# kaftanski/fissure-segmentation

Hardware: AMD Instinct MI355X
Metric: points/sec fwd+bwd DGCNN-seg N=2048 k=20 (higher is better)
Workload: dtype f32

## Files before the change

fissure-segmentation_amd/csrc/edgeconv.hip:

```cpp
#include <type_traits>

#include "edgeconv_internal.h"
#include "knn_internal.h"

namespace {

constexpr int TP = 16;
constexpr int FSG_CSR_SPLIT = 16;
constexpr int TPW = 2;

__global__ __launch_bounds__(1024) void csr_build_kernel(const int32_t *__restrict__ idx, int N, int k,
                                                          int32_t *__restrict__ rowptr, int32_t *__restrict__ col) {
    extern __shared__ int sh[];
    int *hist = sh;
    int *part = sh + N;
    const int b = blockIdx.x, tid = threadIdx.x;
    const long NK = (long)N * k;
    const int32_t *ib = idx + b * NK;
    for (int j = tid; j < N; j += 1024) hist[j] = 0;
    __syncthreads();
    for (long e0 = tid; e0 < NK; e0 += 8 * 1024) {
        int dst[8];
#pragma unroll
        for (int u = 0; u < 8; ++u) dst[u] = (e0 + u * 1024 < NK) ? ib[e0 + u * 1024] : -1;
// ... 380 lines not shown
        cm += red2[2][s2][ch];
    }
    const double mu = n > 0.0 ? bm / n : 0.0;
    double M2 = n > 0.0 ? cm - bm * mu : 0.0;
    M2 = M2 > 0.0 ? M2 : 0.0;
    const double var = n > 0.0 ? M2 / n : 0.0;
    mean_out[c] = (float)mu;
    invstd_out[c] = (float)(1.0 / sqrt(var + (double)eps));
    if (running_mean) {
        const double unbiased = n > 1.0 ? M2 / (n - 1.0) : var;
        running_mean[c] = (float)((1.0 - momentum) * running_mean[c] + momentum * mu);
        running_var[c] = (float)((1.0 - momentum) * running_var[c] + momentum * unbiased);
    }
}

__global__ __launch_bounds__(256) void ec1_apply_kernel(const float *__restrict__ ysel, const float *__restrict__ gamma,
                                                         const float *__restrict__ beta, const float *__restrict__ mean,
                                                         const float *__restrict__ invstd, int N, int Co, float slope,
                                                         float *__restrict__ out, float *__restrict__ out_pm) {
    __shared__ float tile[64][65];
    const int b = blockIdx.x, i0 = blockIdx.y * 64, cg = blockIdx.z;
    const int lane = threadIdx.x & 63, wave = __builtin_amdgcn_readfirstlane(threadIdx.x >> 6);
    const int c = cg * 64 + lane;
    const float g = gamma[c] * invstd[c], sh = beta[c] - mean[c] * g;
    float yv[16];
#pragma unroll
    for (int u = 0; u < 16; ++u) yv[u] = ysel[((long)b * N + min(i0 + wave + 4 * u, N - 1)) * Co + c];
#pragma unroll
    for (int u = 0; u < 16; ++u) {
        const int p = wave + 4 * u, i = i0 + p;
// ... 175 lines not shown
    };
    if (i0 + 64 <= N) rows(std::false_type{});
    else rows(std::true_type{});
    red[0][wave][lane] = sb;
    red[1][wave][lane] = sg;
    __syncthreads();
    if (wave == 0) {
        const long rec = (long)b * gridDim.y + blockIdx.y;
        float *pr = partials + rec * 2 * Co;
        pr[c] = red[0][0][lane] + red[0][1][lane] + red[0][2][lane] + red[0][3][lane];
        pr[Co + c] = red[1][0][lane] + red[1][1][lane] + red[1][2][lane] + red[1][3][lane];
    }
}

constexpr int SUMP_CH = 16, SUMP_SLICES = 64;
__global__ __launch_bounds__(SUMP_CH * SUMP_SLICES) void sum_partials_kernel(const float *__restrict__ partials, int R, int Co,
                                                                             int nvec, float *__restrict__ out0,
                                                                             float *__restrict__ out1) {
    __shared__ double red[SUMP_SLICES][SUMP_CH];
    const int ch = threadIdx.x & (SUMP_CH - 1), slice = threadIdx.x / SUMP_CH;
    const int c = blockIdx.x * SUMP_CH + ch, v = blockIdx.y;
    double acc = 0.0;
    for (int r0 = slice; r0 < R; r0 += 4 * SUMP_SLICES) {
        float t[4];
#pragma unroll
        for (int u = 0; u < 4; ++u) t[u] = partials[((long)min(r0 + u * SUMP_SLICES, R - 1) * nvec + v) * Co + c];
#pragma unroll
        for (int u = 0; u < 4; ++u)
            if (r0 + u * SUMP_SLICES < R) acc += t[u];
    }
    red[slice][ch] = acc;
    __syncthreads();
    if (slice < 8) {
        double t = 0.0;
#pragma unroll
        for (int w = 0; w < 8; ++w) t += red[8 * slice + w][ch];
        red[8 * slice][ch] = t;
    }
    __syncthreads();
    if (slice == 0) {
        double t = 0.0;
#pragma unroll
        for (int w = 0; w < 8; ++w) t += red[8 * w][ch];
        (v == 0 ? out0 : out1)[c] = (float)t;
    }
}

__global__ __launch_bounds__(256) void ec1_bwd_gather_kernel(
    const float *__restrict__ pq, const int32_t *__restrict__ rowptr, const int32_t *__restrict__ col,
    const float *__restrict__ h, const uint8_t *__restrict__ arg, const float *__restrict__ ssum,
    const float *__restrict__ gamma, const float *__restrict__ mean, const float *__restrict__ invstd,
    const float *__restrict__ dbeta, const float *__restrict__ dgamma, int N, int k, int Co, int training, float invM,
    float *__restrict__ grad_pq) {
    typedef f32x2 f2;
    typedef f32x4 f4;
    __shared__ float comb[4][2][4][64];
    const int b = blockIdx.x, cg = blockIdx.z;
    const int lane = threadIdx.x & 63, wave = __builtin_amdgcn_readfirstlane(threadIdx.x >> 6);
    const int j = blockIdx.y * 4 + wave;
    if (j >= N) return;
// ... 64 lines not shown
}

}

int fsg_ec_stats1_records(int B, int N) { return B * fsg_cdiv(N, TP * TPW); }

int fsg_ec_stats1_launch(const float *pq, const int32_t *idx, const float *gamma, int B, int N, int k, int Co,
                         float *ysel, uint8_t *arg, float *ssum, float *partials, hipStream_t st) {
    FSG_REQUIRE((long)N * 2 * Co * 4 < (1L << 31), "edgeconv/stats: a cloud's [P | Q] rows must stay below 2 GiB (N=%d, Co=%d)", N, Co);
    hipLaunchKernelGGL(ec1_stats_select_kernel<false>, dim3(B, fsg_cdiv(N, TP * TPW), Co / 64), dim3(256 * TPW), 0, st, pq, idx,
                       gamma, N, k, Co, 1, ysel, arg, ssum, partials);
    FSG_CHECK_LAUNCH("edgeconv/stats");
    return FSG_OK;
}

size_t fsg_ec_finalize_stage_floats(int Co) { return (size_t)FIN_S * 3 * Co * 2 + 2; }

int fsg_ec_finalize_launch(const float *partials, int R, int Co, float eps, float momentum, float *mean, float *invstd,
                           float *running_mean, float *running_var, hipStream_t st) {
    hipLaunchKernelGGL(bn_finalize_kernel, dim3(Co / FIN_CH), dim3(FIN_CH * FIN_SL), 0, st, partials, R, Co, eps, momentum, mean, invstd,
                       running_mean, running_var);
    FSG_CHECK_LAUNCH("edgeconv/finalize");
    return FSG_OK;
}

int fsg_ec_apply_prep_launch(const float *ysel, const float *gamma, const float *beta, const float *mean, const float *invstd,
                             int B, int N, int Co, float slope, float *out, float *out_pm, void *knn_ws, size_t knn_ws_bytes,
                             const float *w_next, float *pq_next, hipStream_t st) {
    float *xx, *xs, *cscale;
    void *cand;
// ... 237 lines not shown
```

fissure-segmentation_amd/csrc/edgeconv2.hip:

```cpp

#include "edgeconv_internal.h"

namespace {

__device__ __forceinline__ bf16x8 pack8(const float (&v)[8]) {
    bf16x8 r;
#pragma unroll
    for (int i = 0; i < 8; ++i) r[i] = (__bf16)v[i];
    return r;
}

constexpr int C1 = 64;
constexpr int LD1 = C1 + 1;
constexpr int MAXPAIR = 3;

struct Tile {
    int TP, R, Rpad;
};

template <int C2, bool BF>
__global__ __launch_bounds__(256) void ec2_fwd_kernel(const float *__restrict__ pq, const int32_t *__restrict__ idx,
                                                       const float *__restrict__ w2, const float *__restrict__ gamma1,
                                                       const float *__restrict__ beta1, const float *__restrict__ mean1,
                                                       const float *__restrict__ invstd1,
// ... 1060 lines not shown
        { int RTb, TPb, Gb; ec2s_tiling(k, B, N, false, true, RTb, TPb, Gb); if (Gb > Gs) Gs = Gb; }
        if (Gs > G) G = Gs;
    }
    const size_t rec1 = (size_t)fsg_ec_stats1_records(B, N) * 3 * C1 + fsg_ec_finalize_stage_floats(C1);
    const size_t rec2 = (size_t)B * G * 3 * C2 + fsg_ec_finalize_stage_floats(C2);
    const size_t scratch1 = (size_t)B * N * C1 * sizeof(float) + (size_t)B * N * C1;
    return sizeof(float) * (rec1 + rec2) + scratch1 + 256;
}

static int ec2_fwd_impl(bool bf16, const float *pq, const int32_t *idx, const float *w2, const float *gamma1,
                                     const float *beta1, float *running_mean1, float *running_var1, const float *gamma2,
                                     const float *beta2, float *running_mean2, float *running_var2, int B, int N, int k,
                                     int C2, int training, float momentum1, float momentum2, float eps1, float eps2,
                                     float slope, float *out, float *out_pm, float *ssum1, float *mean1, float *invstd1,
                                     float *ysel2, uint8_t *arg2, float *ssum2, float *mean2, float *invstd2,
                                     void *workspace, fsg_stream_t stream) {
    FSG_REQUIRE(pq && idx && w2 && gamma1 && beta1 && gamma2 && beta2 && mean1 && invstd1 && ysel2 && arg2 &&
                    mean2 && invstd2 && workspace,
                "fsg_edgeconv2_fwd_f32: NULL pointer");
    FSG_REQUIRE(B > 0 && N > 0 && N <= (1 << 21) && k > 0 && k <= 64 && (C2 == 64 || C2 == 128) && B <= 65535,
                "fsg_edgeconv2_fwd_f32: bad shape B=%d N=%d k=%d C2=%d (layer widths 64 -> 64|128 only, N <= 2^21)", B, N, k, C2);
    FSG_REQUIRE(!training || (ssum1 && ssum2), "fsg_edgeconv2_fwd_f32: training needs ssum1/ssum2");
    hipStream_t st = (hipStream_t)stream;
    int TP, Rpad, G;
    ec2_tiling(k, C2, TP, Rpad, G, B, N);
    int RTs = 0, TPs = 0, Gs = 0, Gws = G;
    if (ec2_split(C2)) {
        ec2s_tiling(k, B, N, false, bf16, RTs, TPs, Gs);
        if (Gs > Gws) Gws = Gs;
    }
    const int rec1 = fsg_ec_stats1_records(B, N);
    float *part1 = (float *)workspace;
    float *part2 = part1 + (size_t)rec1 * 3 * C1 + fsg_ec_finalize_stage_floats(C1);
    float *ysel1 = part2 + (size_t)B * Gws * 3 * C2 + fsg_ec_finalize_stage_floats(C2);
    uint8_t *arg1 = (uint8_t *)(ysel1 + (size_t)B * N * C1);
    int rc;
    if (training) {
        if ((rc = fsg_ec_stats1_launch(pq, idx, gamma1, B, N, k, C1, ysel1, arg1, ssum1, part1, st)) != FSG_OK) return rc;
        if ((rc = fsg_ec_finalize_launch(part1, rec1, C1, eps1, momentum1, mean1, invstd1, running_mean1, running_var1,
                                         st)) != FSG_OK)
            return rc;
    }
    const size_t lds = sizeof(float) * ((size_t)C2 * LD1 + (size_t)Rpad * (C2 + 1) + 3 * 4 * C2);
#define FSG_EC2_FWD(CC, BFX)                                                                                             \
    do {                                                                                                                 \
        FSG_GRANT_LDS("fsg_edgeconv2_fwd", (ec2_fwd_kernel<CC, BFX>), FSG_LDS_WHOLE_CU);                             \
        hipLaunchKernelGGL((ec2_fwd_kernel<CC, BFX>), dim3(B, G), dim3(256), lds, st, pq, idx, w2, gamma1, beta1, mean1,    \
                           invstd1, gamma2, N, k, TP, Rpad, training, slope, ysel2, arg2, ssum2, part2);                 \
    } while (0)
#define FSG_EC2S_FWD(NPX, RTX)                                                                                            \
    do {                                                                                                                 \
        FSG_GRANT_LDS("fsg_edgeconv2_fwd", (ec2s_fwd_kernel<NPX, RTX>), FSG_LDS_WHOLE_CU);                           \
// ... 24 lines not shown
                                     int C2, int training, float momentum1, float momentum2, float eps1, float eps2,
                                     float slope, float *out, float *out_pm, float *ssum1, float *mean1, float *invstd1,
                                     float *ysel2, uint8_t *arg2, float *ssum2, float *mean2, float *invstd2,
                                     void *workspace, fsg_stream_t stream) {
    return ec2_fwd_impl(false, pq, idx, w2, gamma1, beta1, running_mean1, running_var1, gamma2, beta2, running_mean2, running_var2, B, N, k, C2, training, momentum1, momentum2, eps1, eps2, slope, out, out_pm, ssum1, mean1, invstd1, ysel2, arg2, ssum2, mean2, invstd2, workspace, stream);
}

extern "C" int fsg_edgeconv2_fwd_bf16(const float *pq, const int32_t *idx, const float *w2, const float *gamma1,
                                     const float *beta1, float *running_mean1, float *running_var1, const float *gamma2,
                                     const float *beta2, float *running_mean2, float *running_var2, int B, int N, int k,
                                     int C2, int training, float momentum1, float momentum2, float eps1, float eps2,
                                     float slope, float *out, float *out_pm, float *ssum1, float *mean1, float *invstd1,
                                     float *ysel2, uint8_t *arg2, float *ssum2, float *mean2, float *invstd2,
                                     void *workspace, fsg_stream_t stream) {
    return ec2_fwd_impl(true, pq, idx, w2, gamma1, beta1, running_mean1, running_var1, gamma2, beta2, running_mean2, running_var2, B, N, k, C2, training, momentum1, momentum2, eps1, eps2, slope, out, out_pm, ssum1, mean1, invstd1, ysel2, arg2, ssum2, mean2, invstd2, workspace, stream);
}

static void ec2_bwd_tiling(int k, int C2, int &TP, int &Rpad, int &G, int B, int N) {
    TP = 64 / k;
    if (TP < 1) TP = 1;
    Rpad = (TP * k + 31) & ~31;
    const int ntiles = (N + TP - 1) / TP;
    G = 768 / (B > 0 ? B : 1);
    if (G < 1) G = 1;
    if (G > ntiles) G = ntiles;
}

extern "C" size_t fsg_edgeconv2_bwd_workspace_bytes(int B, int N, int k, int C2) {
    int TP, Rpad, G;
    ec2_bwd_tiling(k, C2, TP, Rpad, G, B, N);
// ... 58 lines not shown
        FSG_GRANT_LDS("fsg_edgeconv2_bwd_f32", (ec2s_bwd_kernel<NPX, RTX>), FSG_LDS_WHOLE_CU);                       \
        hipLaunchKernelGGL((ec2s_bwd_kernel<NPX, RTX>), dim3(B, G), dim3(256), ec2s_bwd_lds(NPX, RTX, TPs), st, pq, idx,   \
                           w2, gamma1, beta1, mean1, invstd1, gamma2, mean2, invstd2, grad_beta2, grad_gamma2, h2, arg2, \
                           N, k, TPs, training, invM, slope, du1, dw_part, p1_part);                                     \
    } while (0)
    if (ec2_split(C2)) {
        G = Gs;
        FSG_REQUIRE(ec2s_bwd_lds(bf16 ? 1 : 3, RTs, TPs) <= FSG_LDS_WHOLE_CU, "fsg_edgeconv2_bwd: k=%d needs too much LDS", k);
        if (bf16) { if (RTs == 4) FSG_EC2S_BWD(1, 4); else FSG_EC2S_BWD(1, 2); }
        else { if (RTs == 4) FSG_EC2S_BWD(3, 4); else FSG_EC2S_BWD(3, 2); }
    } else if (C2 == 64) { if (bf16) FSG_EC2_BWD(64, true); else FSG_EC2_BWD(64, false); }
    else { if (bf16) FSG_EC2_BWD(128, true); else FSG_EC2_BWD(128, false); }
#undef FSG_EC2_BWD
#undef FSG_EC2S_BWD
    FSG_CHECK_LAUNCH("fsg_edgeconv2_bwd_f32/mlp");
    if ((rc = fsg_ec_sum_launch(dw_part, B * G, C2 * C1, 1, grad_w2, nullptr, st)) != FSG_OK) return rc;
    if ((rc = fsg_ec_sum_launch(p1_part, B * G, C1, 2, grad_beta1, grad_gamma1, st)) != FSG_OK) return rc;
    hipLaunchKernelGGL(ec2_bwd_gather_kernel, dim3(B, fsg_cdiv(N, 4)), dim3(256), 0, st, pq, rowptr, col, du1, ssum1,
                       gamma1, mean1, invstd1, grad_beta1, grad_gamma1, N, k, training, invM, grad_pq);
    FSG_CHECK_LAUNCH("fsg_edgeconv2_bwd_f32/gather");
    return FSG_OK;
}

extern "C" int fsg_edgeconv2_bwd_f32(const float *grad_out, const float *grad_out_pm, int64_t ld_pm, const float *grad_out_pm2,
                                     int64_t ld_pm2, const float *pq, const int32_t *idx,
                                     const int32_t *rowptr, const int32_t *col, const float *w2, const float *gamma1,
                                     const float *beta1, const float *mean1, const float *invstd1, const float *ssum1,
                                     const float *gamma2, const float *beta2, const float *mean2, const float *invstd2,
                                     const float *ysel2, const uint8_t *arg2, int B, int N, int k, int C2, int training,
                                     float slope, float *grad_pq, float *grad_w2, float *grad_gamma1, float *grad_beta1,
                                     float *grad_gamma2, float *grad_beta2, void *workspace, fsg_stream_t stream) {
    return ec2_bwd_impl(false, grad_out, grad_out_pm, ld_pm, grad_out_pm2, ld_pm2, pq, idx, rowptr, col, w2, gamma1, beta1, mean1, invstd1, ssum1, gamma2, beta2, mean2, invstd2, ysel2, arg2, B, N, k, C2, training, slope, grad_pq, grad_w2, grad_gamma1, grad_beta1, grad_gamma2, grad_beta2, workspace, stream);
// ... 13 lines not shown
```

fissure-segmentation_amd/csrc/edgeconv_internal.h:

```cpp
#pragma once
#include "fsg_common.h"

int fsg_ec_stats1_records(int B, int N);
int fsg_ec_stats1_launch(const float *pq, const int32_t *idx, const float *gamma, int B, int N, int k, int Co,
                         float *ysel, uint8_t *arg, float *ssum, float *partials, hipStream_t st);
int fsg_ec_apply_launch(const float *ysel, const float *gamma, const float *beta, const float *mean, const float *invstd,
                        int B, int N, int Co, float slope, float *out, float *out_pm, hipStream_t st);
int fsg_ec_apply_prep_launch(const float *ysel, const float *gamma, const float *beta, const float *mean, const float *invstd,
                             int B, int N, int Co, float slope, float *out, float *out_pm, void *knn_ws, size_t knn_ws_bytes,
                             const float *w_next, float *pq_next, hipStream_t st);
int fsg_ec_bwd_point_launch(const float *gout, const float *gout_pm, long ld_pm, const float *gout_pm2, long ld_pm2,
                            const float *ysel, const float *gamma, const float *beta, const float *mean, const float *invstd,
                            int B, int N, int Co, float slope, float *h, float *partials, float *dbeta, float *dgamma,
                            hipStream_t st);

size_t fsg_ec_finalize_stage_floats(int Co);
int fsg_ec_finalize_launch(const float *partials, int R, int Co, float eps, float momentum, float *mean, float *invstd,
                           float *running_mean, float *running_var, hipStream_t st);
int fsg_ec_sum_launch(const float *partials, int R, int L, int nvec, float *out0, float *out1, hipStream_t st);

int fsg_csr_bipartite_launch(const int32_t *idx, int B, int NS, int N, int k, int32_t *rowptr, int32_t *col, int32_t *cnt,
                             int32_t *tmp, hipStream_t st);
```

fissure-segmentation_amd/functional.py:

```python
import contextlib as _contextlib
import ctypes
import os as _os

import torch

from . import _lib


def _need_gpu(*tensors):
    for t in tensors:
        if t is not None and not t.is_cuda:
            raise RuntimeError("fissure_segmentation_amd runs on the GPU only (got a CPU tensor); "
                               "the CPU restatement lives in oracle/ and is test infrastructure")


def _p(t):
    return ctypes.c_void_p(t.data_ptr() if t is not None else 0)


def _stream():
    return ctypes.c_void_p(torch.cuda.current_stream().cuda_stream)


def _f32c(t):
# ... 856 lines not shown
        w_cat = _EdgeWeights.apply(conv_weight.reshape(Co, C2).to(torch.float32))
    if x_pm is None:
        x_pm = x.transpose(1, 2)
    if pq_given is not None:
        pq = _LinearPMGiven.apply(x_pm.to(torch.float32), w_cat, pq_given)
    else:
        pq = linear_pm(x_pm.to(torch.float32).contiguous(), w_cat)
    bn_args = _bn_args(bn)
    if idx.dtype != torch.int32:
        idx = idx.to(torch.int32)
    idx = idx.contiguous()
    res = _EdgeConv1.apply(pq, idx, *bn_args, float(slope), knn_ws, w_next if knn_ws is not None else None)
    return _edgeconv_outputs(res, both, w_next is not None)


class _EdgeConv2(torch.autograd.Function):
    @staticmethod
    @_amp_fwd
    def forward(ctx, pq, idx, w2, g1, b1, rm1, rv1, g2, b2, rm2, rv2, training, mom1, mom2, eps1, eps2, slope, knn_ws=None,
                w_next=None):
        pq, w2 = _f32c(pq), _f32c(w2)
        g1, b1, g2, b2 = _f32c(g1), _f32c(b1), _f32c(g2), _f32c(b2)
        B, N, _ = pq.shape
        C2, k, dev = w2.shape[0], idx.shape[2], pq.device

        def new(*shape, dtype=torch.float32):
            return torch.empty(*shape, dtype=dtype, device=dev)
        out, out_pm = new(B, C2, N), new(B, N, C2)
        ysel2, arg2 = new(B, N, C2), new(B, N, C2, dtype=torch.uint8)
        if training:
            ssum1, ssum2 = new(B, N, 64), new(B, N, C2)
            mean1, invstd1, mean2, invstd2 = new(64), new(64), new(C2), new(C2)
        else:
            ssum1 = ssum2 = None
            mean1, invstd1 = _bn_eval_stats(rm1, rv1, eps1)
            mean2, invstd2 = _bn_eval_stats(rm2, rv2, eps2)
        ws = _lib.workspace("fsg_edgeconv2", B, N, k, C2, device=dev)
        t = bool(training)
        ctx.bf16 = bf16_operands()
        with torch.cuda.device(dev):
            _lib.call("fsg_edgeconv2_fwd_bf16" if ctx.bf16 else "fsg_edgeconv2_fwd_f32", _p(pq), _p(idx), _p(w2), _p(g1), _p(b1),
                      _p(rm1 if t else None),
                      _p(rv1 if t else None), _p(g2), _p(b2), _p(rm2 if t else None), _p(rv2 if t else None), B, N, k, C2,
                      int(t), mom1, mom2, eps1, eps2, slope, _p(None if knn_ws is not None else out), _p(out_pm), _p(ssum1), _p(mean1),
                      _p(invstd1), _p(ysel2), _p(arg2), _p(ssum2), _p(mean2), _p(invstd2), _p(ws), _stream())
            pq_next = _apply_pass(ysel2, g2, b2, mean2, invstd2, B, N, C2, slope, out, out_pm, knn_ws, w_next)
        ctx.save_for_backward(pq, idx, w2, g1, b1, mean1, invstd1, ssum1, g2, b2, mean2, invstd2, ysel2, arg2)
        ctx.meta = (B, N, k, C2, t, slope)
        ctx.set_materialize_grads(False)
        if pq_next is None:
            return out, out_pm, out_pm.view(B, N, C2)
        ctx.mark_non_differentiable(pq_next)
        return out, out_pm, out_pm.view(B, N, C2), pq_next

    @staticmethod
    @_amp_bwd
    def backward(ctx, g, g_pm, g_pm2, _g_pq_next=None):
        pq, idx, w2, g1, b1, mean1, invstd1, ssum1, g2, b2, mean2, invstd2, ysel2, arg2 = ctx.saved_tensors
        B, N, k, C2, training, slope = ctx.meta
        dev = pq.device
        g = _f32c(g) if g is not None else None
        g_pm, ld1 = _pm_grad(g_pm, B, N, C2)
        g_pm2, ld2 = _pm_grad(g_pm2, B, N, C2)
        rowptr, col = reverse_graph(idx)
        gpq, gw2 = torch.empty_like(pq), torch.empty_like(w2)
        dg1, db1 = torch.empty_like(g1), torch.empty_like(b1)
        dg2, db2 = torch.empty_like(g2), torch.empty_like(b2)
        ws = _lib.workspace("fsg_edgeconv2_bwd", B, N, k, C2, device=dev)
        with torch.cuda.device(dev):
            _lib.call("fsg_edgeconv2_bwd_bf16" if ctx.bf16 else "fsg_edgeconv2_bwd_f32", _p(g), _p(g_pm), ld1, _p(g_pm2), ld2,
                      _p(pq), _p(idx), _p(rowptr), _p(col),
                      _p(w2), _p(g1),
                      _p(b1), _p(mean1), _p(invstd1), _p(ssum1), _p(g2), _p(b2), _p(mean2), _p(invstd2), _p(ysel2),
                      _p(arg2), B, N, k, C2, int(training), slope, _p(gpq), _p(gw2), _p(dg1), _p(db1), _p(dg2), _p(db2),
                      _p(ws), _stream())
        return (gpq, None, gw2, dg1, db1, None, None, dg2, db2) + (None,) * 10


def edgeconv2_supported(c_mid, c_out, k):
    return c_mid == 64 and c_out in (64, 128) and k <= 64


def _edgeconv_outputs(res, both, want_pq_next):
    out, out_pm, out_pm2 = res[:3]
    pq_next = res[3] if len(res) > 3 else None
    if both == "twice":
        r = (out, out_pm, out_pm2)
    elif both:
        r = (out, out_pm)
    else:
        r = (out,)
# ... 11 lines not shown
        w_cat = _EdgeWeights.apply(conv1_weight.reshape(C1, CC).to(torch.float32))
    if x_pm is None:
        x_pm = x.transpose(1, 2)
    if pq_given is not None:
        pq = _LinearPMGiven.apply(x_pm.to(torch.float32), w_cat, pq_given)
    else:
        pq = linear_pm(x_pm.to(torch.float32).contiguous(), w_cat)
    w2 = conv2_weight.reshape(conv2_weight.shape[0], C1)
    t1, m1 = _bn_step(bn1)
    t2, m2 = _bn_step(bn2)
    if t1 != t2:
        raise RuntimeError("edgeconv2: both BatchNorm layers must be in the same mode")
    if idx.dtype != torch.int32:
        idx = idx.to(torch.int32)
    idx = idx.contiguous()
    res = _EdgeConv2.apply(pq, idx, w2, bn1.weight, bn1.bias, bn1.running_mean, bn1.running_var,
                           bn2.weight, bn2.bias, bn2.running_mean, bn2.running_var, t1, m1, m2,
                           float(bn1.eps), float(bn2.eps), float(slope), knn_ws, w_next if knn_ws is not None else None)
    return _edgeconv_outputs(res, both, w_next is not None)


def pw_weight_image(w, scale=1.0, out=None, ks0=0, KS=None):
    _need_gpu(w)
    N, K = w.shape
    ks = (K + 15) // 16
    KS = ks if KS is None else KS
    if out is None:
        out = torch.empty(((N + 31) // 32) * KS * 3 * 1024, dtype=torch.uint8, device=w.device)
    with torch.cuda.device(w.device):
        _lib.call("fsg_pw_weight_image_f32", _p(w), w.stride(0), w.stride(1), N, K, float(scale), ks0, KS, _p(out), _stream())
    return out


# ... 3163 lines not shown
```

include/fsg_hip.h:

```cpp
#ifndef FSG_HIP_H
#define FSG_HIP_H

#include <stddef.h>
#include <stdint.h>

#ifdef __cplusplus
extern "C" {
#endif

#define FSG_OK 0
#define FSG_ERR_ARG 1
#define FSG_ERR_HIP 2
#define FSG_ERR_UNSUPPORTED 3

#define FSG_KNN_FIX_DIAG 1
#define FSG_KNN_DROP_FIRST 2

#define FSG_KNN_FORCE_ROWS 4

#define FSG_KNN_FORCE_MFMA 8
#define FSG_KNN_DBG_HALF_CHUNKS (1 << 11)
#define FSG_KNN_DBG_TWO_PHASE (1 << 21)
#define FSG_KNN_DBG_ALL_SLOW (1 << 22)
#define FSG_KNN_DBG_STATS (1 << 25)
// ... 96 lines not shown
int fsg_edgeconv2_bwd_f32(const float *grad_out, const float *grad_out_pm, int64_t ld_pm, const float *grad_out_pm2,
                          int64_t ld_pm2, const float *pq, const int32_t *idx,
                          const int32_t *rowptr, const int32_t *col, const float *w2, const float *gamma1,
                          const float *beta1, const float *mean1, const float *invstd1, const float *ssum1,
                          const float *gamma2, const float *beta2, const float *mean2, const float *invstd2,
                          const float *ysel2, const uint8_t *arg2, int B, int N, int k, int C2, int training,
                          float slope, float *grad_pq, float *grad_w2, float *grad_gamma1, float *grad_beta1,
                          float *grad_gamma2, float *grad_beta2, void *workspace, fsg_stream_t stream);
int fsg_edgeconv2_fwd_bf16(const float *pq, const int32_t *idx, const float *w2, const float *gamma1,
                           const float *beta1, float *running_mean1, float *running_var1, const float *gamma2,
                           const float *beta2, float *running_mean2, float *running_var2, int B, int N, int k, int C2,
                           int training, float momentum1, float momentum2, float eps1, float eps2, float slope,
                           float *out, float *out_pm, float *ssum1, float *mean1, float *invstd1, float *ysel2,
                           uint8_t *arg2, float *ssum2, float *mean2, float *invstd2, void *workspace,
                           fsg_stream_t stream);
int fsg_edgeconv2_bwd_bf16(const float *grad_out, const float *grad_out_pm, int64_t ld_pm, const float *grad_out_pm2,
                           int64_t ld_pm2, const float *pq, const int32_t *idx,
                           const int32_t *rowptr, const int32_t *col, const float *w2, const float *gamma1,
                           const float *beta1, const float *mean1, const float *invstd1, const float *ssum1,
                           const float *gamma2, const float *beta2, const float *mean2, const float *invstd2,
                           const float *ysel2, const uint8_t *arg2, int B, int N, int k, int C2, int training,
                           float slope, float *grad_pq, float *grad_w2, float *grad_gamma1, float *grad_beta1,
                           float *grad_gamma2, float *grad_beta2, void *workspace, fsg_stream_t stream);

size_t fsg_bn_act_workspace_bytes(long M, int C);
int fsg_bn_act_fwd_f32(const float *y, const float *gamma, const float *beta, float *running_mean, float *running_var,
                       long M, int C, int training, float momentum, float eps, float slope, float *out, float *mean,
                       float *invstd, float *workspace, fsg_stream_t stream);
int fsg_bn_act_bwd_f32(const float *grad_out, const float *y, const float *gamma, const float *beta, const float *mean,
                       const float *invstd, long M, int C, int training, float slope, float *grad_y, float *grad_gamma,
// ... 511 lines not shown
```

Measured before the change: 18.33 million.

## Compute first EdgeConv BN stats from raw-input moments instead of edge features

For the first EdgeConv layer with at most 4 input channels, batch-norm mean and variance are now derived analytically from first and second moments of the raw coordinates over neighbour edges, folded through the linear weights, instead of being reduced over the full 64-channel edge features. A new moments kernel accumulates these moments in double precision (optionally staging the cloud in LDS) and also writes the per-point neighbour sums, and a single-block fold kernel produces mean, invstd and running stats. Separately, the backward partial-sum launches are merged into one paired kernel. This trades a wide channel reduction for a small moment computation, but relies on BN input being exactly linear in x and adds a single-block serial fold.

```diff
diff --git a/fissure-segmentation_amd/csrc/edgeconv.hip b/fissure-segmentation_amd/csrc/edgeconv.hip
--- a/fissure-segmentation_amd/csrc/edgeconv.hip
+++ b/fissure-segmentation_amd/csrc/edgeconv.hip
@@ -418,6 +418,264 @@
     }
 }
 
+constexpr int MOM_THREADS = 256, MOM_LPP = 4, MOM_PTS = MOM_THREADS / MOM_LPP;
+constexpr int MOM_NM = 44;
+constexpr int MOM_ROW = 23;
+constexpr int MOM_FOLD = 11 * MOM_NM + MOM_NM;
+__constant__ unsigned char MOM_IA[MOM_NM] = {0, 1, 2, 3, 18, 19, 20, 21, 4, 5, 6, 7, 8, 9, 10, 11, 12, 13,
+                                             0, 0, 0, 0, 1, 1, 1, 1, 2, 2, 2, 2, 3, 3, 3, 3,
+                                             18, 18, 18, 18, 19, 19, 19, 20, 20, 21};
+__constant__ unsigned char MOM_IB[MOM_NM] = {22, 22, 22, 22, 22, 22, 22, 22, 22, 22, 22, 22, 22, 22, 22, 22, 22, 22,
+                                             14, 15, 16, 17, 14, 15, 16, 17, 14, 15, 16, 17, 14, 15, 16, 17,
+                                             14, 15, 16, 17, 15, 16, 17, 16, 17, 17};
+__device__ __forceinline__ int mom_tri(int a, int b) {
+    return a * 4 - a * (a - 1) / 2 + (b - a);
+}
+
+struct MomentFold {
+    const float *w_cat;
+    int C, R;
+    double edges, inv_edges, k;
+    float eps, momentum;
+    float *mean, *invstd, *running_mean, *running_var;
+};
+
+__device__ __forceinline__ void ec2_moments_fold(const MomentFold &F, const double *rec, double *sh) {
+    typedef double f64x2 __attribute__((ext_vector_type(2)));
+    const int t = threadIdx.x, pm = t % 22, q = t / 22;
+    float wf[8] = {0.f, 0.f, 0.f, 0.f, 0.f, 0.f, 0.f, 0.f}, rm0 = 0.f, rv0 = 0.f;
+    if (t < 64) {
+#pragma unroll
+        for (int a = 0; a < 4; ++a) {
+            const float wa = F.w_cat[(long)t * F.C + min(a, F.C - 1)], wb = F.w_cat[(long)(64 + t) * F.C + min(a, F.C - 1)];
+            wf[a] = a < F.C ? wa : 0.f;
+            wf[4 + a] = a < F.C ? wb : 0.f;
+        }
+        if (F.running_mean) {
+            rm0 = F.running_mean[t];
+            rv0 = F.running_var[t];
+        }
+    }
+    if (q < 11) {
+        double a0 = 0.0, a1 = 0.0;
+        const int r0 = (int)((long)F.R * q / 11), r1 = (int)((long)F.R * (q + 1) / 11);
+        constexpr int RB = 24;
+        for (int r = r0; r < r1; r += RB) {
+            f64x2 v[RB];
+#pragma unroll
+            for (int u = 0; u < RB; ++u)
+                v[u] = *reinterpret_cast<const f64x2 *>(rec + (long)min(r + u, r1 - 1) * MOM_NM + 2 * pm);
+#pragma unroll
+            for (int u = 0; u < RB; ++u)
+                if (r + u < r1) {
+                    a0 += v[u][0];
+                    a1 += v[u][1];
+                }
+        }
+        sh[q * MOM_NM + 2 * pm] = a0;
+        sh[q * MOM_NM + 2 * pm + 1] = a1;
+    }
+    __syncthreads();
+    if (t < MOM_NM) {
+        double a = 0.0;
+#pragma unroll
+        for (int u = 0; u < 11; ++u) a += sh[u * MOM_NM + t];
+        sh[11 * MOM_NM + t] = a;
+    }
+    __syncthreads();
+    if (t >= 64) return;
+    const double *tot = sh + 11 * MOM_NM;
+    const int c = t;
+    double w[8], mf[8];
+#pragma unroll
+    for (int a = 0; a < 4; ++a) {
+        w[a] = (double)wf[a];
+        w[4 + a] = (double)wf[4 + a];
+        mf[a] = tot[a] * F.inv_edges;
+        mf[4 + a] = F.k * tot[4 + a] * F.inv_edges;
+    }
+    double mu = 0.0, var = 0.0;
+#pragma unroll
+    for (int a = 0; a < 8; ++a) mu += w[a] * mf[a];
+#pragma unroll
+    for (int a = 0; a < 8; ++a)
+#pragma unroll
+        for (int b = 0; b < 8; ++b) {
+            double sff;
+            if (a < 4 && b < 4) sff = tot[8 + mom_tri(min(a, b), max(a, b))];
+            else if (a >= 4 && b >= 4) sff = F.k * tot[34 + mom_tri(min(a, b) - 4, max(a, b) - 4)];
+            else sff = tot[18 + 4 * min(a, b) + (max(a, b) - 4)];
+            var += w[a] * w[b] * (sff * F.inv_edges - mf[a] * mf[b]);
+        }
+    var = var > 0.0 ? var : 0.0;
+    F.mean[c] = (float)mu;
+    F.invstd[c] = (float)(1.0 / sqrt(var + (double)F.eps));
+    if (F.running_mean) {
+        const double n = F.edges, unbiased = n > 1.0 ? var * n / (n - 1.0) : var;
+        F.running_mean[c] = (float)((1.0 - F.momentum) * rm0 + F.momentum * mu);
+        F.running_var[c] = (float)((1.0 - F.momentum) * rv0 + F.momentum * unbiased);
+    }
+}
+
+constexpr size_t MOM_LDS_FIXED = sizeof(double) * (MOM_THREADS * MOM_ROW + 4 * 64);
+template <bool STAGE>
+__global__ __launch_bounds__(MOM_THREADS) void ec2_moments_kernel(const float *__restrict__ x, long sb, long sc,
+                                                                  const int32_t *__restrict__ idx,
+                                                                  const float *__restrict__ pq, int N, int k,
+                                                                  float *__restrict__ ssum, double *__restrict__ rec,
+                                                                  const MomentFold F) {
+    typedef f32x4 f4;
+    extern __shared__ __align__(16) unsigned char mom_lds[];
+    double(*row)[MOM_ROW] = reinterpret_cast<double(*)[MOM_ROW]>(mom_lds);
+    double *red = reinterpret_cast<double *>(mom_lds) + MOM_THREADS * MOM_ROW;
+    f4 *cx = reinterpret_cast<f4 *>(mom_lds + MOM_LDS_FIXED);
+    int32_t *ids = reinterpret_cast<int32_t *>(cx + N);
+    const int tid = threadIdx.x, b = blockIdx.y, i0 = blockIdx.x * MOM_PTS, C = F.C;
+    const int p = tid / MOM_LPP, h = tid % MOM_LPP, i = i0 + p;
+    const bool live = i < N;
+    const float *xb = x + (long)b * sb;
+    const int c16 = tid & 15, pg = tid >> 4;
+    const float *qb = pq + (long)b * N * 128 + 64 + 4 * c16;
+    f4 qv[MOM_PTS / 16];
+#pragma unroll
+    for (int u = 0; u < MOM_PTS / 16; ++u) qv[u] = *reinterpret_cast<const f4 *>(qb + (long)min(i0 + 16 * u + pg, N - 1) * 128);
+    float wpf[4][4];
+#pragma unroll
+    for (int e = 0; e < 4; ++e)
+#pragma unroll
+        for (int a = 0; a < 4; ++a) {
+            const float wv = F.w_cat[(long)(4 * c16 + e) * C + min(a, C - 1)];
+            wpf[e][a] = a < C ? wv : 0.f;
+        }
+    double s[4] = {0.0, 0.0, 0.0, 0.0}, T[10] = {0.0, 0.0, 0.0, 0.0, 0.0, 0.0, 0.0, 0.0, 0.0, 0.0};
+    float xi[4] = {0.f, 0.f, 0.f, 0.f};
+    auto add = [&](const float (&v)[4]) {
+        int t = 0;
+#pragma unroll
+        for (int a = 0; a < 4; ++a) {
+            s[a] += (double)v[a];
+#pragma unroll
+            for (int c = a; c < 4; ++c, ++t) T[t] += (double)v[a] * (double)v[c];
+        }
+    };
+    if (STAGE) {
+        constexpr int ICH = MOM_PTS * 64 / MOM_THREADS;
+        constexpr int SCH = 8;
+        const int cnt = min(MOM_PTS, N - i0) * k;
+        const int32_t *it = idx + ((long)b * N + i0) * k;
+        int32_t idv[ICH];
+#pragma unroll
+        for (int u = 0; u < ICH; ++u) idv[u] = tid + u * MOM_THREADS < cnt ? it[tid + u * MOM_THREADS] : 0;
+        for (int n0 = 0; n0 < N; n0 += SCH * MOM_THREADS) {
+            f4 cv[SCH];
+#pragma unroll
+            for (int u = 0; u < SCH; ++u) {
+                const int n = min(n0 + u * MOM_THREADS + tid, N - 1);
+#pragma unroll
+                for (int c = 0; c < 4; ++c) {
+                    const float xv = xb[min(c, C - 1) * sc + n];
+                    cv[u][c] = c < C ? xv : 0.f;
+                }
+            }
+#pragma unroll
+            for (int u = 0; u < SCH; ++u)
+                if (n0 + u * MOM_THREADS + tid < N) cx[n0 + u * MOM_THREADS + tid] = cv[u];
+        }
+#pragma unroll
+        for (int u = 0; u < ICH; ++u)
+            if (tid + u * MOM_THREADS < cnt) ids[tid + u * MOM_THREADS] = idv[u];
+        __syncthreads();
+        if (live) {
+            const f4 v = cx[i];
+#pragma unroll
+            for (int c = 0; c < 4; ++c) xi[c] = v[c];
+#pragma unroll 4
+            for (int sl = h; sl < k; sl += MOM_LPP) {
+                const f4 vj = cx[min(max(ids[p * k + sl], 0), N - 1)];
+                const float xj[4] = {vj[0], vj[1], vj[2], vj[3]};
+                add(xj);
+            }
+        }
+    } else if (live) {
+#pragma unroll
+        for (int c = 0; c < 4; ++c) {
+            const float xv = xb[min(c, C - 1) * sc + i];
+            xi[c] = c < C ? xv : 0.f;
+        }
+        const int32_t *ib = idx + ((long)b * N + i) * k;
+        constexpr int RB = 5;
+        for (int s0 = h; s0 < k; s0 += MOM_LPP * RB) {
+            int j[RB];
+            float xj[RB][4];
+#pragma unroll
+            for (int u = 0; u < RB; ++u) j[u] = min(max(ib[min(s0 + MOM_LPP * u, k - 1)], 0), N - 1);
+#pragma unroll
+            for (int u = 0; u < RB; ++u)
+#pragma unroll
+                for (int c = 0; c < 4; ++c) {
+                    const float xv = xb[min(c, C - 1) * sc + j[u]];
+                    xj[u][c] = c < C ? xv : 0.f;
+                }
+#pragma unroll
+            for (int u = 0; u < RB; ++u)
+                if (s0 + MOM_LPP * u < k) add(xj[u]);
+        }
+    }
+#pragma unroll
+    for (int a = 0; a < 4; ++a) {
+        row[tid][a] = s[a];
+        row[tid][14 + a] = (double)xi[a];
+        row[tid][18 + a] = h == 0 ? (double)xi[a] : 0.0;
+    }
+#pragma unroll
+    for (int t = 0; t < 10; ++t) row[tid][4 + t] = T[t];
+    row[tid][22] = live ? 1.0 : 0.0;
+    __syncthreads();
+    {
+        const int m = tid & 63, q = tid >> 6;
+        double acc = 0.0;
+        if (m < MOM_NM) {
+            const int ia = MOM_IA[m], ibb = MOM_IB[m];
+#pragma unroll 8
+            for (int l = 64 * q; l < 64 * q + 64; ++l) acc += row[l][ia] * row[l][ibb];
+        }
+        red[q * 64 + m] = acc;
+    }
+    __syncthreads();
+    const long r = (long)b * gridDim.x + blockIdx.x;
+    if (tid < MOM_NM) rec[r * MOM_NM + tid] = ((red[tid] + red[64 + tid]) + red[128 + tid]) + red[192 + tid];
+    {
+        float *sb_out = ssum + (long)b * N * 64 + 4 * c16;
+#pragma unroll
+        for (int u = 0; u < MOM_PTS / 16; ++u) {
+            const int pp = 16 * u + pg;
+            if (i0 + pp < N) {
+                double si[4];
+#pragma unroll
+                for (int a = 0; a < 4; ++a) {
+                    si[a] = row[MOM_LPP * pp][a];
+#pragma unroll
+                    for (int l = 1; l < MOM_LPP; ++l) si[a] += row[MOM_LPP * pp + l][a];
+                }
+                f4 o;
+#pragma unroll
+                for (int e = 0; e < 4; ++e) {
+                    double v = (double)k * (double)qv[u][e];
+#pragma unroll
+                    for (int a = 0; a < 4; ++a) v += (double)wpf[e][a] * si[a];
+                    o[e] = (float)v;
+                }
+                *reinterpret_cast<f4 *>(sb_out + (long)(i0 + pp) * 64) = o;
+            }
+        }
+    }
+}
+
+__global__ __launch_bounds__(MOM_THREADS) void ec2_moments_fold_kernel(const double *__restrict__ rec, const MomentFold F) {
+    __shared__ double red[MOM_FOLD];
+    ec2_moments_fold(F, rec, red);
+}
+
 __global__ __launch_bounds__(256) void ec1_apply_kernel(const float *__restrict__ ysel, const float *__restrict__ gamma,
                                                          const float *__restrict__ beta, const float *__restrict__ mean,
                                                          const float *__restrict__ invstd, int N, int Co, float slope,
@@ -623,36 +881,50 @@
 }
 
 constexpr int SUMP_CH = 16, SUMP_SLICES = 64;
+__device__ __forceinline__ void sum_partials_block(const float *__restrict__ partials, int R, int Co, int nvec,
+                                                   float *__restrict__ out0, float *__restrict__ out1, int bx, int v) {
+    __shared__ double red[SUMP_SLICES][SUMP_CH];
+    const int ch = threadIdx.x & (SUMP_CH - 1), slice = threadIdx.x / SUMP_CH;
+    const int c = bx * SUMP_CH + ch;
+    double acc = 0.0;
+    for (int r0 = slice; r0 < R; r0 += 4 * SUMP_SLICES) {
+        float t[4];
+#pragma unroll
+        for (int u = 0; u < 4; ++u) t[u] = partials[((long)min(r0 + u * SUMP_SLICES, R - 1) * nvec + v) * Co + c];
+#pragma unroll
+        for (int u = 0; u < 4; ++u)
+            if (r0 + u * SUMP_SLICES < R) acc += t[u];
+    }
+    red[slice][ch] = acc;
+    __syncthreads();
+    if (slice < 8) {
+        double t = 0.0;
+#pragma unroll
+        for (int w = 0; w < 8; ++w) t += red[8 * slice + w][ch];
+        red[8 * slice][ch] = t;
+    }
+    __syncthreads();
+    if (slice == 0) {
+        double t = 0.0;
+#pragma unroll
+        for (int w = 0; w < 8; ++w) t += red[8 * w][ch];
+        (v == 0 ? out0 : out1)[c] = (float)t;
+    }
+}
+
 __global__ __launch_bounds__(SUMP_CH * SUMP_SLICES) void sum_partials_kernel(const float *__restrict__ partials, int R, int Co,
                                                                              int nvec, float *__restrict__ out0,
                                                                              float *__restrict__ out1) {
-    __shared__ double red[SUMP_SLICES][SUMP_CH];
-    const int ch = threadIdx.x & (SUMP_CH - 1), slice = threadIdx.x / SUMP_CH;
-    const int c = blockIdx.x * SUMP_CH + ch, v = blockIdx.y;
-    double acc = 0.0;
-    for (int r0 = slice; r0 < R; r0 += 4 * SUMP_SLICES) {
-        float t[4];
-#pragma unroll
-        for (int u = 0; u < 4; ++u) t[u] = partials[((long)min(r0 + u * SUMP_SLICES, R - 1) * nvec + v) * Co + c];
-#pragma unroll
-        for (int u = 0; u < 4; ++u)
-            if (r0 + u * SUMP_SLICES < R) acc += t[u];
-    }
-    red[slice][ch] = acc;
-    __syncthreads();
-    if (slice < 8) {
-        double t = 0.0;
-#pragma unroll
-        for (int w = 0; w < 8; ++w) t += red[8 * slice + w][ch];
-        red[8 * slice][ch] = t;
-    }
-    __syncthreads();
-    if (slice == 0) {
-        double t = 0.0;
-#pragma unroll
-        for (int w = 0; w < 8; ++w) t += red[8 * w][ch];
-        (v == 0 ? out0 : out1)[c] = (float)t;
-    }
+    sum_partials_block(partials, R, Co, nvec, out0, out1, blockIdx.x, blockIdx.y);
+}
+
+__global__ __launch_bounds__(SUMP_CH * SUMP_SLICES) void sum_partials_pair_kernel(
+    const float *__restrict__ pa, int Ra, int La, float *__restrict__ out_a, const float *__restrict__ pb, int Rb, int Lb,
+    float *__restrict__ out_b0, float *__restrict__ out_b1) {
+    const int na = La / SUMP_CH, nb = Lb / SUMP_CH;
+    const int bx = blockIdx.x;
+    if (bx < na) sum_partials_block(pa, Ra, La, 1, out_a, nullptr, bx, 0);
+    else sum_partials_block(pb, Rb, Lb, 2, out_b0, out_b1, (bx - na) % nb, (bx - na) / nb);
 }
 
 __global__ __launch_bounds__(256) void ec1_bwd_gather_kernel(
@@ -747,6 +1019,38 @@
     return FSG_OK;
 }
 
+size_t fsg_ec_moments1_record_bytes(int B, int N) { return (size_t)B * fsg_cdiv(N, MOM_PTS) * MOM_NM * sizeof(double); }
+
+int fsg_ec_moments1_launch(const float *x, long sb, long sc, int C, const int32_t *idx, const float *w_cat, const float *pq, int B,
+                           int N, int k, float eps, float momentum, float *ssum, float *mean, float *invstd, float *running_mean,
+                           float *running_var, void *records, hipStream_t st) {
+    const dim3 grid(fsg_cdiv(N, MOM_PTS), B);
+    const double edges = (double)B * (double)N * (double)k;
+    const MomentFold F{w_cat, C, (int)(grid.x * grid.y), edges, 1.0 / edges, (double)k, eps, momentum,
+                       mean, invstd, running_mean, running_var};
+    const size_t staged = MOM_LDS_FIXED + 16 * (size_t)N + 4 * (size_t)MOM_PTS * k;
+    if (staged <= FSG_LDS_WHOLE_CU) {
+        FSG_GRANT_LDS("fsg_edgeconv2_fwd_moments", ec2_moments_kernel<true>, staged);
+        hipLaunchKernelGGL(ec2_moments_kernel<true>, grid, dim3(MOM_THREADS), staged, st, x, sb, sc, idx, pq, N, k, ssum,
+                           (double *)records, F);
+    } else {
+        hipLaunchKernelGGL(ec2_moments_kernel<false>, grid, dim3(MOM_THREADS), MOM_LDS_FIXED, st, x, sb, sc, idx, pq, N, k, ssum,
+                           (double *)records, F);
+    }
+    FSG_CHECK_LAUNCH("edgeconv2/moments");
+    hipLaunchKernelGGL(ec2_moments_fold_kernel, dim3(1), dim3(MOM_THREADS), 0, st, (const double *)records, F);
+    FSG_CHECK_LAUNCH("edgeconv2/moments_fold");
+    return FSG_OK;
+}
+
+int fsg_ec_sum_pair_launch(const float *pa, int Ra, int La, float *out_a, const float *pb, int Rb, int Lb, float *out_b0,
+                           float *out_b1, hipStream_t st) {
+    hipLaunchKernelGGL(sum_partials_pair_kernel, dim3(La / SUMP_CH + 2 * (Lb / SUMP_CH)), dim3(SUMP_CH * SUMP_SLICES), 0, st, pa, Ra,
+                       La, out_a, pb, Rb, Lb, out_b0, out_b1);
+    FSG_CHECK_LAUNCH("edgeconv/sum_pair");
+    return FSG_OK;
+}
+
 size_t fsg_ec_finalize_stage_floats(int Co) { return (size_t)FIN_S * 3 * Co * 2 + 2; }
 
 int fsg_ec_finalize_launch(const float *partials, int R, int Co, float eps, float momentum, float *mean, float *invstd,
diff --git a/fissure-segmentation_amd/csrc/edgeconv2.hip b/fissure-segmentation_amd/csrc/edgeconv2.hip
--- a/fissure-segmentation_amd/csrc/edgeconv2.hip
+++ b/fissure-segmentation_amd/csrc/edgeconv2.hip
@@ -1098,7 +1098,8 @@
                                      int C2, int training, float momentum1, float momentum2, float eps1, float eps2,
                                      float slope, float *out, float *out_pm, float *ssum1, float *mean1, float *invstd1,
                                      float *ysel2, uint8_t *arg2, float *ssum2, float *mean2, float *invstd2,
-                                     void *workspace, fsg_stream_t stream) {
+                                     void *workspace, fsg_stream_t stream, const float *x = nullptr, int64_t x_sb = 0,
+                                     int64_t x_sc = 0, int Cx = 0, const float *w_cat = nullptr) {
     FSG_REQUIRE(pq && idx && w2 && gamma1 && beta1 && gamma2 && beta2 && mean1 && invstd1 && ysel2 && arg2 &&
                     mean2 && invstd2 && workspace,
                 "fsg_edgeconv2_fwd_f32: NULL pointer");
@@ -1119,7 +1120,13 @@
     float *ysel1 = part2 + (size_t)B * Gws * 3 * C2 + fsg_ec_finalize_stage_floats(C2);
     uint8_t *arg1 = (uint8_t *)(ysel1 + (size_t)B * N * C1);
     int rc;
-    if (training) {
+    if (training && x && w_cat && Cx >= 1 && Cx <= 4) {
+        FSG_REQUIRE(x_sb >= 0 && x_sc >= 0 && fsg_ec_moments1_record_bytes(B, N) <= sizeof(float) * (size_t)rec1 * 3 * C1,
+                    "fsg_edgeconv2_fwd_moments: bad coordinate strides %ld, %ld", (long)x_sb, (long)x_sc);
+        if ((rc = fsg_ec_moments1_launch(x, (long)x_sb, (long)x_sc, Cx, idx, w_cat, pq, B, N, k, eps1, momentum1, ssum1, mean1,
+                                         invstd1, running_mean1, running_var1, part1, st)) != FSG_OK)
+            return rc;
+    } else if (training) {
         if ((rc = fsg_ec_stats1_launch(pq, idx, gamma1, B, N, k, C1, ysel1, arg1, ssum1, part1, st)) != FSG_OK) return rc;
         if ((rc = fsg_ec_finalize_launch(part1, rec1, C1, eps1, momentum1, mean1, invstd1, running_mean1, running_var1,
                                          st)) != FSG_OK)
@@ -1174,6 +1181,39 @@
                                      float *ysel2, uint8_t *arg2, float *ssum2, float *mean2, float *invstd2,
                                      void *workspace, fsg_stream_t stream) {
     return ec2_fwd_impl(true, pq, idx, w2, gamma1, beta1, running_mean1, running_var1, gamma2, beta2, running_mean2, running_var2, B, N, k, C2, training, momentum1, momentum2, eps1, eps2, slope, out, out_pm, ssum1, mean1, invstd1, ysel2, arg2, ssum2, mean2, invstd2, workspace, stream);
+}
+
+extern "C" int fsg_edgeconv2_fwd_moments_f32(const float *pq, const int32_t *idx, const float *w2, const float *gamma1,
+                                     const float *beta1, float *running_mean1, float *running_var1, const float *gamma2,
+                                     const float *beta2, float *running_mean2, float *running_var2, int B, int N, int k,
+                                     int C2, int training, float momentum1, float momentum2, float eps1, float eps2,
+                                     float slope, float *out, float *out_pm, float *ssum1, float *mean1, float *invstd1,
+                                     float *ysel2, uint8_t *arg2, float *ssum2, float *mean2, float *invstd2,
+                                     const float *x, int64_t x_stride_b, int64_t x_stride_c, int Cx, const float *w_cat,
+                                     void *workspace, fsg_stream_t stream) {
+    return ec2_fwd_impl(false, pq, idx, w2, gamma1, beta1, running_mean1, running_var1, gamma2, beta2, running_mean2, running_var2, B, N, k, C2, training, momentum1, momentum2, eps1, eps2, slope, out, out_pm, ssum1, mean1, invstd1, ysel2, arg2, ssum2, mean2, invstd2, workspace, stream, x, x_stride_b, x_stride_c, Cx, w_cat);
+}
+
+extern "C" int fsg_edgeconv2_fwd_moments_bf16(const float *pq, const int32_t *idx, const float *w2, const float *gamma1,
+                                     const float *beta1, float *running_mean1, float *running_var1, const float *gamma2,
+                                     const float *beta2, float *running_mean2, float *running_var2, int B, int N, int k,
+                                     int C2, int training, float momentum1, float momentum2, float eps1, float eps2,
+                                     float slope, float *out, float *out_pm, float *ssum1, float *mean1, float *invstd1,
+                                     float *ysel2, uint8_t *arg2, float *ssum2, float *mean2, float *invstd2,
+                                     const float *x, int64_t x_stride_b, int64_t x_stride_c, int Cx, const float *w_cat,
+                                     void *workspace, fsg_stream_t stream) {
+    return ec2_fwd_impl(true, pq, idx, w2, gamma1, beta1, running_mean1, running_var1, gamma2, beta2, running_mean2, running_var2, B, N, k, C2, training, momentum1, momentum2, eps1, eps2, slope, out, out_pm, ssum1, mean1, invstd1, ysel2, arg2, ssum2, mean2, invstd2, workspace, stream, x, x_stride_b, x_stride_c, Cx, w_cat);
+}
+
+extern "C" int fsg_edgeconv2_bwd_sums_f32(const float *dw_part, const float *p1_part, int R, int C2, float *grad_w2,
+                                          float *grad_beta1, float *grad_gamma1, int one_launch, fsg_stream_t stream) {
+    FSG_REQUIRE(dw_part && p1_part && grad_w2 && grad_beta1 && grad_gamma1 && R > 0 && (C2 == 64 || C2 == 128),
+                "fsg_edgeconv2_bwd_sums_f32: NULL pointer or bad shape R=%d C2=%d", R, C2);
+    hipStream_t st = (hipStream_t)stream;
+    if (one_launch) return fsg_ec_sum_pair_launch(dw_part, R, C2 * C1, grad_w2, p1_part, R, C1, grad_beta1, grad_gamma1, st);
+    int rc;
+    if ((rc = fsg_ec_sum_launch(dw_part, R, C2 * C1, 1, grad_w2, nullptr, st)) != FSG_OK) return rc;
+    return fsg_ec_sum_launch(p1_part, R, C1, 2, grad_beta1, grad_gamma1, st);
 }
 
 static void ec2_bwd_tiling(int k, int C2, int &TP, int &Rpad, int &G, int B, int N) {
@@ -1262,8 +1302,8 @@
 #undef FSG_EC2_BWD
 #undef FSG_EC2S_BWD
     FSG_CHECK_LAUNCH("fsg_edgeconv2_bwd_f32/mlp");
-    if ((rc = fsg_ec_sum_launch(dw_part, B * G, C2 * C1, 1, grad_w2, nullptr, st)) != FSG_OK) return rc;
-    if ((rc = fsg_ec_sum_launch(p1_part, B * G, C1, 2, grad_beta1, grad_gamma1, st)) != FSG_OK) return rc;
+    if ((rc = fsg_ec_sum_pair_launch(dw_part, B * G, C2 * C1, grad_w2, p1_part, B * G, C1, grad_beta1, grad_gamma1, st)) != FSG_OK)
+        return rc;
     hipLaunchKernelGGL(ec2_bwd_gather_kernel, dim3(B, fsg_cdiv(N, 4)), dim3(256), 0, st, pq, rowptr, col, du1, ssum1,
                        gamma1, mean1, invstd1, grad_beta1, grad_gamma1, N, k, training, invM, grad_pq);
     FSG_CHECK_LAUNCH("fsg_edgeconv2_bwd_f32/gather");
diff --git a/fissure-segmentation_amd/csrc/edgeconv_internal.h b/fissure-segmentation_amd/csrc/edgeconv_internal.h
--- a/fissure-segmentation_amd/csrc/edgeconv_internal.h
+++ b/fissure-segmentation_amd/csrc/edgeconv_internal.h
@@ -4,6 +4,10 @@
 int fsg_ec_stats1_records(int B, int N);
 int fsg_ec_stats1_launch(const float *pq, const int32_t *idx, const float *gamma, int B, int N, int k, int Co,
                          float *ysel, uint8_t *arg, float *ssum, float *partials, hipStream_t st);
+size_t fsg_ec_moments1_record_bytes(int B, int N);
+int fsg_ec_moments1_launch(const float *x, long sb, long sc, int C, const int32_t *idx, const float *w_cat, const float *pq, int B,
+                           int N, int k, float eps, float momentum, float *ssum, float *mean, float *invstd, float *running_mean,
+                           float *running_var, void *records, hipStream_t st);
 int fsg_ec_apply_launch(const float *ysel, const float *gamma, const float *beta, const float *mean, const float *invstd,
                         int B, int N, int Co, float slope, float *out, float *out_pm, hipStream_t st);
 int fsg_ec_apply_prep_launch(const float *ysel, const float *gamma, const float *beta, const float *mean, const float *invstd,
@@ -18,6 +22,8 @@
 int fsg_ec_finalize_launch(const float *partials, int R, int Co, float eps, float momentum, float *mean, float *invstd,
                            float *running_mean, float *running_var, hipStream_t st);
 int fsg_ec_sum_launch(const float *partials, int R, int L, int nvec, float *out0, float *out1, hipStream_t st);
+int fsg_ec_sum_pair_launch(const float *pa, int Ra, int La, float *out_a, const float *pb, int Rb, int Lb, float *out_b0,
+                           float *out_b1, hipStream_t st);
 
 int fsg_csr_bipartite_launch(const int32_t *idx, int B, int NS, int N, int k, int32_t *rowptr, int32_t *col, int32_t *cnt,
                              int32_t *tmp, hipStream_t st);
diff --git a/fissure-segmentation_amd/functional.py b/fissure-segmentation_amd/functional.py
--- a/fissure-segmentation_amd/functional.py
+++ b/fissure-segmentation_amd/functional.py
@@ -894,11 +894,20 @@
     return _edgeconv_outputs(res, both, w_next is not None)
 
 
+_ec2_moment_stats = True
+
+
+def set_ec2_moment_stats(flag):
+    global _ec2_moment_stats
+    old, _ec2_moment_stats = _ec2_moment_stats, bool(flag)
+    return old
+
+
 class _EdgeConv2(torch.autograd.Function):
     @staticmethod
     @_amp_fwd
     def forward(ctx, pq, idx, w2, g1, b1, rm1, rv1, g2, b2, rm2, rv2, training, mom1, mom2, eps1, eps2, slope, knn_ws=None,
-                w_next=None):
+                w_next=None, x_mom=None, w_mom=None):
         pq, w2 = _f32c(pq), _f32c(w2)
         g1, b1, g2, b2 = _f32c(g1), _f32c(b1), _f32c(g2), _f32c(b2)
         B, N, _ = pq.shape
@@ -918,12 +927,15 @@
         ws = _lib.workspace("fsg_edgeconv2", B, N, k, C2, device=dev)
         t = bool(training)
         ctx.bf16 = bf16_operands()
+        extras = ()
+        if t and x_mom is not None and w_mom is not None:
+            extras = (_p(x_mom), x_mom.stride(0), x_mom.stride(1), x_mom.shape[1], _p(w_mom))
         with torch.cuda.device(dev):
-            _lib.call("fsg_edgeconv2_fwd_bf16" if ctx.bf16 else "fsg_edgeconv2_fwd_f32", _p(pq), _p(idx), _p(w2), _p(g1), _p(b1),
-                      _p(rm1 if t else None),
+            _lib.call("fsg_edgeconv2_fwd" + ("_moments" if extras else "") + ("_bf16" if ctx.bf16 else "_f32"), _p(pq), _p(idx),
+                      _p(w2), _p(g1), _p(b1), _p(rm1 if t else None),
                       _p(rv1 if t else None), _p(g2), _p(b2), _p(rm2 if t else None), _p(rv2 if t else None), B, N, k, C2,
                       int(t), mom1, mom2, eps1, eps2, slope, _p(None if knn_ws is not None else out), _p(out_pm), _p(ssum1), _p(mean1),
-                      _p(invstd1), _p(ysel2), _p(arg2), _p(ssum2), _p(mean2), _p(invstd2), _p(ws), _stream())
+                      _p(invstd1), _p(ysel2), _p(arg2), _p(ssum2), _p(mean2), _p(invstd2), *extras, _p(ws), _stream())
             pq_next = _apply_pass(ysel2, g2, b2, mean2, invstd2, B, N, C2, slope, out, out_pm, knn_ws, w_next)
         ctx.save_for_backward(pq, idx, w2, g1, b1, mean1, invstd1, ssum1, g2, b2, mean2, invstd2, ysel2, arg2)
         ctx.meta = (B, N, k, C2, t, slope)
@@ -954,7 +966,7 @@
                       _p(b1), _p(mean1), _p(invstd1), _p(ssum1), _p(g2), _p(b2), _p(mean2), _p(invstd2), _p(ysel2),
                       _p(arg2), B, N, k, C2, int(training), slope, _p(gpq), _p(gw2), _p(dg1), _p(db1), _p(dg2), _p(db2),
                       _p(ws), _stream())
-        return (gpq, None, gw2, dg1, db1, None, None, dg2, db2) + (None,) * 10
+        return (gpq, None, gw2, dg1, db1, None, None, dg2, db2) + (None,) * 12
 
 
 def edgeconv2_supported(c_mid, c_out, k):
@@ -996,9 +1008,16 @@
     if idx.dtype != torch.int32:
         idx = idx.to(torch.int32)
     idx = idx.contiguous()
+    x_mom = w_mom = None
+    if _ec2_moment_stats and t1 and C <= 4 and x.dim() == 3 and tuple(w_cat.shape) == (2 * C1, C):
+        x_mom = x.detach()
+        if x_mom.dtype != torch.float32 or x_mom.stride(2) != 1 or x_mom.data_ptr() % 4:
+            x_mom = x_mom.float().contiguous()
+        w_mom = _f32c(w_cat.detach())
     res = _EdgeConv2.apply(pq, idx, w2, bn1.weight, bn1.bias, bn1.running_mean, bn1.running_var,
                            bn2.weight, bn2.bias, bn2.running_mean, bn2.running_var, t1, m1, m2,
-                           float(bn1.eps), float(bn2.eps), float(slope), knn_ws, w_next if knn_ws is not None else None)
+                           float(bn1.eps), float(bn2.eps), float(slope), knn_ws, w_next if knn_ws is not None else None,
+                           x_mom, w_mom)
     return _edgeconv_outputs(res, both, w_next is not None)
 
 
diff --git a/include/fsg_hip.h b/include/fsg_hip.h
--- a/include/fsg_hip.h
+++ b/include/fsg_hip.h
@@ -134,6 +134,24 @@
                            float *out, float *out_pm, float *ssum1, float *mean1, float *invstd1, float *ysel2,
                            uint8_t *arg2, float *ssum2, float *mean2, float *invstd2, void *workspace,
                            fsg_stream_t stream);
+int fsg_edgeconv2_fwd_moments_f32(const float *pq, const int32_t *idx, const float *w2, const float *gamma1,
+                                  const float *beta1, float *running_mean1, float *running_var1, const float *gamma2,
+                                  const float *beta2, float *running_mean2, float *running_var2, int B, int N, int k, int C2,
+                                  int training, float momentum1, float momentum2, float eps1, float eps2, float slope,
+                                  float *out, float *out_pm, float *ssum1, float *mean1, float *invstd1, float *ysel2,
+                                  uint8_t *arg2, float *ssum2, float *mean2, float *invstd2, const float *x,
+                                  int64_t x_stride_b, int64_t x_stride_c, int Cx, const float *w_cat, void *workspace,
+                                  fsg_stream_t stream);
+int fsg_edgeconv2_fwd_moments_bf16(const float *pq, const int32_t *idx, const float *w2, const float *gamma1,
+                                   const float *beta1, float *running_mean1, float *running_var1, const float *gamma2,
+                                   const float *beta2, float *running_mean2, float *running_var2, int B, int N, int k, int C2,
+                                   int training, float momentum1, float momentum2, float eps1, float eps2, float slope,
+                                   float *out, float *out_pm, float *ssum1, float *mean1, float *invstd1, float *ysel2,
+                                   uint8_t *arg2, float *ssum2, float *mean2, float *invstd2, const float *x,
+                                   int64_t x_stride_b, int64_t x_stride_c, int Cx, const float *w_cat, void *workspace,
+                                   fsg_stream_t stream);
+int fsg_edgeconv2_bwd_sums_f32(const float *dw_part, const float *p1_part, int R, int C2, float *grad_w2, float *grad_beta1,
+                               float *grad_gamma1, int one_launch, fsg_stream_t stream);
 int fsg_edgeconv2_bwd_bf16(const float *grad_out, const float *grad_out_pm, int64_t ld_pm, const float *grad_out_pm2,
                            int64_t ld_pm2, const float *pq, const int32_t *idx,
                            const int32_t *rowptr, const int32_t *col, const float *w2, const float *gamma1,
```

Result: no change. 18.35 million (median of 4 runs) (+0.1%).
